# arielmission-space/PAOS

Measured on AMD Instinct MI355X. Metric: wavefronts/sec (4096^2 c128, 20-surface chain) + achieved HBM GB/s, higher is better.
Workload: dtype c128 (f64); 1 GPU; SYN20 20-surface chain (SURVEY 8d: 43 2-D FFTs per wavefront as the reference runs it), 4096x4096 fp64, walked 512-wavelength sweep, 32 wavefronts/GPU/step, PSFs stay in HBM; separable pass programs + ptp identities ([24] passes/wavefront, parity 1e-15..2e-14 vs oracle); grid=4096, batch_per_gpu=32, parallelism=wavefront-sharded x1, transport=none (single process), ranks_seen=1, launcher=none

## Files before the change

### include/paos_hip.h

```cpp
#ifndef PAOS_HIP_H
#define PAOS_HIP_H

#ifdef __cplusplus
extern "C" {
#endif

typedef struct paos_ctx paos_ctx;

enum { PAOS_OK = 0, PAOS_EINVAL = 1, PAOS_EHIP = 2, PAOS_EUNSUPPORTED = 3 };
enum { PAOS_F64 = 0, PAOS_F32 = 1 };
enum { PAOS_SHAPE_ELLIPSE = 0, PAOS_SHAPE_RECT = 1 };
enum { PAOS_KERNEL_PASS_ROWS = 0, PAOS_KERNEL_PASS_COLS = 1, PAOS_KERNEL_PASS_ANY = 2 };
enum { PAOS_PW_SIGN = 1, PAOS_PW_QPHASE_CENTRED = 2, PAOS_PW_QPHASE_NATURAL = 3, PAOS_PW_SCALE = 4,
       PAOS_PW_MASK = 5 };
enum { PAOS_PWF_MUL2PI = 1,
       PAOS_PWF_X_ONLY = 2, PAOS_PWF_Y_ONLY = 4 };
enum { PAOS_MAX_PW = 6 };
enum { PAOS_NORM_SLOTS = 64 };
enum { PAOS_WHAT_FIELD = 0, PAOS_WHAT_AMPLITUDE = 1, PAOS_WHAT_PHASE = 2, PAOS_WHAT_INTENSITY = 3 };

enum { PAOS_PHASE_STRIDE = 5 };
enum { PAOS_APERTURE_STRIDE = 8 };
enum { PAOS_ZERNIKE_HEAD = 8 };

// ... 75 lines not shown
int paos_focus_begin(paos_ctx* ctx);
int paos_focus_plane(paos_ctx* ctx, const double* params);
int paos_focus_end(paos_ctx* ctx);
enum { PAOS_OTF_MTF = 0, PAOS_OTF_COMPLEX = 1 };
int paos_otf_compute(paos_ctx* ctx);
int paos_otf_fetch(paos_ctx* ctx, int item, int what, void* host_out);
int paos_otf_cuts(paos_ctx* ctx, double* host_out);
int paos_zoom_weights(int n, int s, double frac, double* w, int* carry);
enum { PAOS_ZOOM_PSF = 0, PAOS_ZOOM_FIELD = 1 };
int paos_zoom_compute(paos_ctx* ctx, int m, int s, const double* centres, int want_field);
int paos_zoom_fetch(paos_ctx* ctx, int item, int what, void* host_out);
int paos_run_passes(paos_ctx* ctx, const paos_pass* passes, int n_passes, const double* blocks,
                    int n_blocks);
int paos_copy_yardstick(paos_ctx* ctx, int reps, double* ms_per_launch, double* bytes_per_launch);
int paos_record_set_stats(paos_ctx* ctx, unsigned long long* found, unsigned long long* rendered);
int paos_ctx_set_pruning(paos_ctx* ctx, int on);
int paos_run_passes_live(paos_ctx* ctx, const paos_pass* passes, int n_passes, const double* blocks,
                         int n_blocks, const double* live_rows);
int paos_run_program(paos_ctx* ctx, const paos_pass* passes, int n_passes, const double* blocks, int n_blocks,
                     const paos_program_opts* opts);
int paos_zernike(paos_ctx* ctx, int nmax, int kdim, const double* table, const double* params,
                 int param_stride, double* host_wfe);
int paos_zernike_like(paos_ctx* ctx, int nmax, int kdim, const double* table, const double* params,
                      int param_stride, const double* same_as, double* host_wfe);


int paos_pupil_aperture(paos_ctx* ctx, int shape, const double* params);
int paos_pupil_upload(paos_ctx* ctx, int item, const double* host_weights);
int paos_zernike_gram(paos_ctx* ctx, int nmax, int kdim, const double* table, const double* params,
                      int param_stride, int K, const double* poly, int use_pupil, double* host_out);
// ... 19 lines not shown
```

### paos_amd/_lib.py

```python
import ctypes
import os
import threading
import weakref

import numpy as np

_HERE = os.path.dirname(os.path.abspath(__file__))
LIB_PATH = os.environ.get("PAOS_LIB") or os.path.join(_HERE, "libpaoship.so")

PAOS_F64, PAOS_F32 = 0, 1
SHAPE_ELLIPSE, SHAPE_RECT = 0, 1
WHAT_FIELD, WHAT_AMPLITUDE, WHAT_PHASE, WHAT_INTENSITY = 0, 1, 2, 3
KERNEL_PASS_ROWS, KERNEL_PASS_COLS, KERNEL_PASS_ANY = 0, 1, 2
PW_SIGN, PW_QPHASE_CENTRED, PW_QPHASE_NATURAL, PW_SCALE, PW_MASK = 1, 2, 3, 4, 5
PWF_MUL2PI = 1
PWF_X_ONLY, PWF_Y_ONLY = 2, 4
MAX_PW = 6
OTF_MTF, OTF_COMPLEX = 0, 1
ZOOM_PSF, ZOOM_FIELD = 0, 1
ZOOM_MAX_TABLES = 256
NORM_SLOTS = 64


class PwOp(ctypes.Structure):
# ... 50 lines not shown
    "paos_ptp": (ctypes.c_int, [_c_ctx, _dbl_p]),
    "paos_stw": (ctypes.c_int, [_c_ctx, _dbl_p, ctypes.c_int]),
    "paos_wts": (ctypes.c_int, [_c_ctx, _dbl_p, ctypes.c_int]),
    "paos_focus_begin": (ctypes.c_int, [_c_ctx]),
    "paos_focus_plane": (ctypes.c_int, [_c_ctx, _dbl_p]),
    "paos_focus_end": (ctypes.c_int, [_c_ctx]),
    "paos_otf_compute": (ctypes.c_int, [_c_ctx]),
    "paos_otf_fetch": (ctypes.c_int, [_c_ctx, ctypes.c_int, ctypes.c_int, ctypes.c_void_p]),
    "paos_otf_cuts": (ctypes.c_int, [_c_ctx, _dbl_p]),
    "paos_zoom_weights": (ctypes.c_int, [ctypes.c_int, ctypes.c_int, ctypes.c_double, _dbl_p, ctypes.POINTER(ctypes.c_int)]),
    "paos_zoom_compute": (ctypes.c_int, [_c_ctx, ctypes.c_int, ctypes.c_int, _dbl_p, ctypes.c_int]),
    "paos_zoom_fetch": (ctypes.c_int, [_c_ctx, ctypes.c_int, ctypes.c_int, ctypes.c_void_p]),
    "paos_run_passes": (ctypes.c_int, [_c_ctx, ctypes.POINTER(Pass), ctypes.c_int, _dbl_p, ctypes.c_int]),
    "paos_copy_yardstick": (ctypes.c_int, [_c_ctx, ctypes.c_int, _dbl_p, _dbl_p]),
    "paos_record_set_stats": (ctypes.c_int, [_c_ctx, ctypes.POINTER(ctypes.c_ulonglong), ctypes.POINTER(ctypes.c_ulonglong)]),
    "paos_ctx_set_pruning": (ctypes.c_int, [_c_ctx, ctypes.c_int]),
    "paos_run_passes_live": (ctypes.c_int, [_c_ctx, ctypes.POINTER(Pass), ctypes.c_int, _dbl_p, ctypes.c_int, _dbl_p]),
    "paos_zernike": (ctypes.c_int, [_c_ctx, ctypes.c_int, ctypes.c_int, _dbl_p, _dbl_p, ctypes.c_int, _dbl_p]),
    "paos_psf_keep": (ctypes.c_int, [_c_ctx]),
    "paos_psf_keep_power": (ctypes.c_int, [_c_ctx, ctypes.POINTER(ctypes.c_int)]),
    "paos_psf_fetch": (ctypes.c_int, [_c_ctx, ctypes.c_int, _dbl_p]),
    "paos_host_alloc": (ctypes.c_int, [ctypes.c_ulonglong, ctypes.POINTER(ctypes.c_void_p)]),
    "paos_host_free": (ctypes.c_int, [ctypes.c_void_p]),
    "paos_export_pinned": (ctypes.c_int, [_c_ctx, ctypes.c_int, ctypes.c_int, ctypes.c_void_p]),
    "paos_start": (ctypes.c_int, [_c_ctx, ctypes.c_double, ctypes.c_double, ctypes.c_int, _dbl_p, _dbl_p]),
    "paos_pupil_aperture": (ctypes.c_int, [_c_ctx, ctypes.c_int, _dbl_p]),
    "paos_pupil_upload": (ctypes.c_int, [_c_ctx, ctypes.c_int, _dbl_p]),
    "paos_zernike_like": (ctypes.c_int, [_c_ctx, ctypes.c_int, ctypes.c_int, _dbl_p, _dbl_p, ctypes.c_int, _dbl_p, _dbl_p]),
    "paos_zernike_gram": (ctypes.c_int, [_c_ctx, ctypes.c_int, ctypes.c_int, _dbl_p, _dbl_p, ctypes.c_int,
                                         ctypes.c_int, _dbl_p, ctypes.c_int, _dbl_p]),
# ... 496 lines not shown
                                              out.ctypes.data_as(ctypes.c_void_p)), "paos_zoom_fetch")
        return out

    def copy_yardstick(self, reps=10):
        ms, nbytes = ctypes.c_double(0.0), ctypes.c_double(0.0)
        self._check(self._lib.paos_copy_yardstick(self._ctx, int(reps), ctypes.byref(ms), ctypes.byref(nbytes)),
                    "paos_copy_yardstick")
        return ms.value, nbytes.value

    def record_set_stats(self):
        found, rendered = ctypes.c_ulonglong(0), ctypes.c_ulonglong(0)
        self._check(self._lib.paos_record_set_stats(self._ctx, ctypes.byref(found), ctypes.byref(rendered)),
                    "paos_record_set_stats")
        return int(found.value), int(rendered.value)

    def set_pruning(self, on):
        self._check(self._lib.paos_ctx_set_pruning(self._ctx, 1 if on else 0), "paos_ctx_set_pruning")

    def run_passes(self, passes, blocks, live_rows=None, rows_stale=False, final_intensity=False, live_cols=None):
        b = np.ascontiguousarray(blocks, dtype=np.float64)
        if b.ndim != 3 or b.shape[1:] != (self.batch, PHASE_STRIDE):
            raise ValueError("blocks must be [n_blocks][batch][5]")
        arr = (Pass * len(passes))()
        for dst, src in zip(arr, passes):
            dst.axis, dst.fft1, dst.fft2 = src["axis"], src.get("fft1", -1), src.get("fft2", -1)
            for name in ("pre", "mid", "post"):
                ops = src.get(name, ())
                if len(ops) > MAX_PW:
                    raise ValueError("too many operators in one pass slot")
                setattr(dst, "n_" + name, len(ops))
# ... 108 lines not shown
```

### paos_amd/csrc/context.hip

```cpp
#include "host.h"

#include <cmath>
#include <complex>
#include <cstring>
#include <mutex>
#include <set>
#include <utility>

namespace {

thread_local std::string g_err;

}

int fail(paos_ctx* c, int code, const std::string& msg) {
  if (c) c->err = msg;
  g_err = msg;
  return code;
}

namespace {

int arena_switch(paos_ctx* c) {
  Arena& a = c->arena;
// ... 219 lines not shown
  c->device = device; c->n = n; c->batch = batch; c->precision = precision;
  const int bc = precision == PAOS_F64 ? Lay<double>::BC : Lay<float>::BC;
  c->br = (precision == PAOS_F32 && n >= 2048) ? PAOS_F32_BR : PAOS_BR;
  c->pitch = (unsigned)n * c->br + (unsigned)PAOS_PAD_BLOCKS * c->br * bc;
  c->item_stride = c->pitch * (unsigned)(n / c->br);
  const size_t eb = elem_bytes(c);
  auto bail = [&](hipError_t e, const char* what) {
    std::string msg = std::string(what) + ": " + hipGetErrorString(e);
    paos_ctx_destroy(c);
    return fail(nullptr, PAOS_EHIP, msg);
  };
  hipError_t e;
  if ((e = hipSetDevice(device)) != hipSuccess) return bail(e, "hipSetDevice");
  if ((e = hipStreamCreateWithFlags(&c->stream, hipStreamNonBlocking)) != hipSuccess) return bail(e, "hipStreamCreate");
  if (const char* pad = getenv("PAOS_LDS_PAD")) c->lds_pad = (size_t)std::max(0, std::atoi(pad));
  if ((e = hipMalloc(&c->dyn_scale, (size_t)batch * sizeof(double))) != hipSuccess) return bail(e, "hipMalloc(dyn_scale)");
  {
    std::vector<double> ones((size_t)batch, 1.0);
    if ((e = hipMemcpy(c->dyn_scale, ones.data(), ones.size() * sizeof(double), hipMemcpyHostToDevice)) != hipSuccess) return bail(e, "hipMemcpy(dyn_scale)");
  }
  if ((e = hipMalloc(&c->field, (size_t)c->item_stride * batch * eb)) != hipSuccess) return bail(e, "hipMalloc(field)");
  if ((e = hipMemsetAsync(c->field, 0, (size_t)c->item_stride * batch * eb, c->stream)) != hipSuccess) return bail(e, "hipMemset(field)");
  if ((e = hipMalloc(&c->tw, (size_t)n * eb)) != hipSuccess) return bail(e, "hipMalloc(tw)");
  if ((e = hipMalloc(&c->staging, (size_t)n * n * 16)) != hipSuccess) return bail(e, "hipMalloc(staging)");
  c->nparts = 1024;
  if ((e = hipMalloc(&c->partial, (size_t)batch * c->nparts * sizeof(double))) != hipSuccess) return bail(e, "hipMalloc(partial)");
  if ((e = hipMalloc(&c->norm2, (size_t)batch * sizeof(double))) != hipSuccess) return bail(e, "hipMalloc(norm2)");
  if ((e = hipHostMalloc(&c->norm2_host, (size_t)kNormSlots * batch * sizeof(double))) != hipSuccess) return bail(e, "hipHostMalloc(norm2)");
  c->arena.cap = (size_t)1 << 18;
  if (c->arena.cap < (size_t)batch * 2048) c->arena.cap = (size_t)batch * 2048;
// ... 165 lines not shown
}

int paos_norm2_release(paos_ctx* c, int ticket) {
  if (!c || ticket < 0 || ticket >= kNormSlots) return fail(c, PAOS_EINVAL, "bad ticket");
  c->norm_busy[ticket] = false;
  return PAOS_OK;
}

int paos_record_set_stats(paos_ctx* c, unsigned long long* found, unsigned long long* rendered) {
  if (!c || !found || !rendered) return fail(c, PAOS_EINVAL, "bad record-set request");
  *found = c->mask_hits;
  *rendered = c->mask_rendered;
  return PAOS_OK;
}

int paos_ctx_set_pruning(paos_ctx* c, int on) {
  if (!c) return fail(c, PAOS_EINVAL, "null context");
  c->prune = on != 0;
  return PAOS_OK;
}

}
```

### paos_amd/csrc/fft_core.h

```cpp
#pragma once
#include <hip/hip_runtime.h>

namespace paos {

template <typename T>
struct cx {
  T x, y;
};

template <typename T>
__device__ __forceinline__ cx<T> cadd(cx<T> a, cx<T> b) { return {a.x + b.x, a.y + b.y}; }
template <typename T>
__device__ __forceinline__ cx<T> csub(cx<T> a, cx<T> b) { return {a.x - b.x, a.y - b.y}; }
template <typename T>
__device__ __forceinline__ cx<T> cmul(cx<T> a, cx<T> b) {
  return {fma(a.x, b.x, -(a.y * b.y)), fma(a.x, b.y, a.y * b.x)};
}
template <typename T>
__device__ __forceinline__ cx<T> cconj(cx<T> a) { return {a.x, -a.y}; }
template <typename T>
__device__ __forceinline__ cx<T> sub_ib(cx<T> a, cx<T> b) { return {a.x + b.y, a.y - b.x}; }
template <typename T>
__device__ __forceinline__ cx<T> add_ib(cx<T> a, cx<T> b) { return {a.x - b.y, a.y + b.x}; }
template <typename T>
// ... 183 lines not shown
    dft<4, DIR>(b);
#pragma unroll
    for (int k2 = 0; k2 < 4; ++k2) v[4 * k2] = b[k2];
  }
  lf_twiddled_dft4<1, DIR>(y + 4, o);
#pragma unroll
  for (int k2 = 0; k2 < 4; ++k2) v[1 + 4 * k2] = o[k2];
  lf_twiddled_dft4<2, DIR>(y + 8, o);
#pragma unroll
  for (int k2 = 0; k2 < 4; ++k2) v[2 + 4 * k2] = o[k2];
  lf_twiddled_dft4<3, DIR>(y + 12, o);
#pragma unroll
  for (int k2 = 0; k2 < 4; ++k2) v[3 + 4 * k2] = o[k2];
}

template <int R, int DIR, typename T>
__device__ __forceinline__ void dft(cx<T>* v) {
  if constexpr (R == 16 && PAOS_LF16 != 0) {
    dft16_lf<DIR>(v);
  } else if constexpr (R == 2) {
    cx<T> a = v[0], b = v[1];
    v[0] = cadd(a, b);
    v[1] = csub(a, b);
  } else if constexpr (R == 4) {
    cx<T> t0 = cadd(v[0], v[2]), t1 = csub(v[0], v[2]);
    cx<T> t2 = cadd(v[1], v[3]), t3 = csub(v[1], v[3]);
    v[0] = cadd(t0, t2);
    v[2] = csub(t0, t2);
    if constexpr (DIR > 0) {
      v[1] = sub_ib(t1, t3);
// ... 89 lines not shown
#endif
#define PAOS_SYNC() do { if (!(PAOS_DIAG & 1)) __syncthreads(); } while (0)
#define PAOS_SYNC_X() do { if (!((PAOS_DIAG & 4) && NS > 1)) PAOS_SYNC(); } while (0)

#define PAOS_FENCE() do { if constexpr (FR != 0) __builtin_amdgcn_sched_barrier(0); } while (0)
#ifndef PAOS_NOFENCE
#define PAOS_NOFENCE 0
#endif
#define PAOS_FENCE_IF(bit) do { if constexpr (FR != 0 && !(PAOS_NOFENCE & (bit))) __builtin_amdgcn_sched_barrier(0); } while (0)
#ifndef PAOS_TAIL_FENCE
#define PAOS_TAIL_FENCE 1
#endif
#ifndef PAOS_TABLE_TWIDDLES
#define PAOS_TABLE_TWIDDLES 1
#endif
template <typename T, int N, int E, int DIR, bool SPLIT, int NS = 1, int FR = 0>
__device__ __forceinline__ void fft_stages(cx<T>* v, void* lds, int t,
                                           const cx<T>* __restrict__ tw, const cx<double>* circle = nullptr,
                                           const cx<T>* w1_last = nullptr) {
  using S = StageInfo<N, E, NS>;
  constexpr int TL = N / E;
  constexpr int R = S::R;
  constexpr int TPT = S::TPT;

#pragma unroll
  for (int s = 0; s < TPT; ++s) {
    if constexpr (NS > 1) {
      const int j = t + s * TL;
      const int k = j & (NS - 1);
      if constexpr (FR != 0 && PAOS_TABLE_TWIDDLES && sizeof(T) == 8 && NS * R == 256) {
        cx<double> wa = circle[k], wb = circle[2 * k];
// ... 1 lines not shown
        for (int r = 1; r < R; ++r) {
          const cx<double> w = wa;
          wa = wb;
          if (r + 2 < R) wb = circle[k * (r + 2)];
          v[s * R + r] = cmul(v[s * R + r], cx<T>{(T)w.x, (T)(DIR > 0 ? -w.y : w.y)});
          PAOS_FENCE_IF(4);
        }
      } else {
        cx<T> w1 = (w1_last != nullptr && NS * R == N) ? w1_last[s] : tw[k * (N / (NS * R))];
        if constexpr (DIR < 0) w1.y = -w1.y;
        if constexpr (FR != 0) apply_twiddle_chain<R>(v + s * R, w1);
        else apply_twiddle_powers<R>(v + s * R, w1);
      }
      PAOS_FENCE_IF(2);
    }
    if constexpr (!(((PAOS_DIAG & 8) && NS == 1) || ((PAOS_DIAG & 16) && S::LAST))) dft<R, DIR>(v + s * R);
    if constexpr (!(S::LAST && PAOS_TAIL_FENCE == 0)) PAOS_FENCE();
  }

  if constexpr (!S::LAST) {
    using SN = StageInfo<N, E, NS * R>;
    constexpr int R2 = SN::R;
    constexpr int TPT2 = SN::TPT;
    constexpr bool LIN_R = (TL % 16 == 0) && ((N / R2) % 16 == 0);
    int wb[TPT];
#pragma unroll
    for (int s = 0; s < TPT; ++s) {
      const int j = t + s * TL;
      wb[s] = lds_pad((j / NS) * (NS * R) + (j & (NS - 1)));
    }
    const int rb = lds_pad(t);
// ... 24 lines not shown
            if (!(PAOS_DIAG & 2)) l[wb[s] + lds_pad(r * NS)] = part ? v[s * R + r].y : v[s * R + r].x;
        PAOS_SYNC_X();
#pragma unroll
        for (int s = 0; s < TPT2; ++s)
#pragma unroll
          for (int r = 0; r < R2; ++r) {
            if (!(PAOS_DIAG & 2)) {
              const T val = l[ridx(s, r)];
              if (part) v[s * R2 + r].y = val; else v[s * R2 + r].x = val;
            }
          }
        if (part == 0 || !SN::LAST) PAOS_SYNC_X();
      }
    }
    PAOS_FENCE_IF(1);
    fft_stages<T, N, E, DIR, SPLIT, NS * R, FR>(v, lds, t, tw, circle, w1_last);
  }
}

constexpr int kSwapRow = 272;

__device__ __forceinline__ int swap_nibbles(int t) { return ((t & 15) << 4) | (t >> 4); }

template <typename T, bool BARRIER>
__device__ __forceinline__ void swap_exchange(cx<T>* v, T* lds, int wbase, int wstride, int rbase, int rstride, bool first) {
#pragma unroll
  for (int part = 0; part < 2; ++part) {
    if (BARRIER && (part == 1 || !first)) __syncthreads();
#pragma unroll
    for (int r = 0; r < 16; ++r) lds[wbase + r * wstride] = part ? v[r].y : v[r].x;
    if (BARRIER) __syncthreads();
// ... 75 lines not shown
```

### paos_amd/csrc/frugal_launch.h

```cpp
#pragma once
#include "host.h"

namespace {

#ifndef PAOS_LONG_ONE_LINE
#define PAOS_LONG_ONE_LINE 1
#endif
#ifndef PAOS_SINGLE_ONE_LINE
#define PAOS_SINGLE_ONE_LINE 1
#endif
template <typename T, int N, int AXIS, int KPRE, int KMID, int NFFT, int STORE = 0, int TAB = 0, int LONG = 0, int ONE = 0>
int frugal_launch(paos_ctx* c, const FrugalArgs& args) {
  using C = FftCfg<T, N>;
  constexpr bool kOneLine = PAOS_LONG_ONE_LINE != 0 && (LONG != 0 || ONE != 0) && STORE == 0 && sizeof(T) == 8 && N == 4096;
  constexpr int kOcc = (PAOS_LONG_ONE_LINE != 0 && (LONG != 0 || ONE != 0) && STORE == 0 && sizeof(T) == 8 && N == 2048) ? 1 : 0;
  constexpr int LINES = kOneLine ? 1 : (AXIS == 0 ? C::FR_ROW_LINES : C::COL_LINES);
  constexpr int TILES = AXIS == 0 ? C::ROW_TILES : C::COL_TILES;
  constexpr bool SPLIT = sizeof(T) == 8 || LINES > 2;
  FrugalArgs a = args;
  unsigned groups = N / LINES / TILES;
  a.wg0 = 0;
  constexpr unsigned kAlign = (kOneLine && AXIS == 0) ? 32 : 16;
  static_assert((N / LINES / TILES) % kAlign == 0, "TileMap renumbers tiles inside aligned groups of workgroups");
  if (a.live_hi > a.live_lo) {
    const unsigned per = LINES * TILES;
    a.wg0 = (a.live_lo / per) / kAlign * kAlign;
    unsigned end = ((a.live_hi + per - 1) / per + kAlign - 1) / kAlign * kAlign;
    if (end > groups) end = groups;
    groups = end - a.wg0;
  }
  const dim3 grid(groups, c->batch), block(TILES * LINES * N / C::E);
  constexpr size_t kMaxPad = 8192;
  const size_t lds = frugal_lds_bytes<T, N, LINES, TILES, SPLIT, KPRE, KMID, C::E, STORE, kOcc>() + (c->lds_pad < kMaxPad ? c->lds_pad : kMaxPad);
  auto kern = frugal_pass_kernel<T, N, C::E, LINES, TILES, AXIS, C::BR, C::BC, SPLIT, KPRE, KMID, NFFT, STORE, TAB, LONG, kOcc>;
  return TIMED_LAUNCH(c, kern, grid, block, lds, frugal_lds_bytes<T, N, LINES, TILES, SPLIT, KPRE, KMID, C::E, STORE, kOcc>() + kMaxPad,
                      AXIS == 0 ? PAOS_KERNEL_PASS_ROWS : PAOS_KERNEL_PASS_COLS, c->prof_next_tag, PAOS_FRUGAL_PASS(a));
}

template <typename T, int N, int AXIS, int KPRE, int KMID>
int frugal_nfft(paos_ctx* c, const FrugalArgs& a, int nfft) {
  if (a.tab && a.fuse) {
    if constexpr (KPRE == 1 && KMID == 1) {
      if (nfft < 2) return fail(c, PAOS_EINVAL, "a fused chain starts with a two-transform pass");
#define PAOS_LONG_CASE(L)                                                           \
  case L:                                                                           \
    if (a.psf) return frugal_launch<T, N, AXIS, 1, 1, 2, 1, 1, L>(c, a);            \
    if (a.pow_partial) return frugal_launch<T, N, AXIS, 1, 1, 2, 2, 1, L>(c, a);    \
    return frugal_launch<T, N, AXIS, 1, 1, 2, 0, 1, L>(c, a);
      switch (a.fuse) {
        PAOS_LONG_CASE(1)
        PAOS_LONG_CASE(2)
        PAOS_LONG_CASE(3)
        PAOS_LONG_CASE(4)
      }
#undef PAOS_LONG_CASE
      return fail(c, PAOS_EINVAL, "a launch runs at most three passes");
    } else {
      return fail(c, PAOS_EINVAL, "no fused build of this pass shape");
    }
  }
  if (a.tab) {
    if constexpr (KPRE <= 1 && KMID <= 1 && KPRE + KMID > 0) {
      if (a.psf) return nfft >= 2 ? frugal_launch<T, N, AXIS, KPRE, KMID, 2, 1, 1>(c, a) : frugal_launch<T, N, AXIS, KPRE, KMID, 1, 1, 1>(c, a);
      if (a.pow_partial) return nfft >= 2 ? frugal_launch<T, N, AXIS, KPRE, KMID, 2, 2, 1>(c, a) : frugal_launch<T, N, AXIS, KPRE, KMID, 1, 2, 1>(c, a);
      if constexpr (sizeof(T) == 8 && (N == 4096 || N == 2048) && PAOS_LONG_ONE_LINE != 0) {
        if (a.one_line && PAOS_SINGLE_ONE_LINE != 0) return nfft >= 2 ? frugal_launch<T, N, AXIS, KPRE, KMID, 2, 0, 1, 0, 1>(c, a) : frugal_launch<T, N, AXIS, KPRE, KMID, 1, 0, 1, 0, 1>(c, a);
      }
      return nfft >= 2 ? frugal_launch<T, N, AXIS, KPRE, KMID, 2, 0, 1>(c, a) : frugal_launch<T, N, AXIS, KPRE, KMID, 1, 0, 1>(c, a);
    } else {
      return fail(c, PAOS_EINVAL, "no table build of this pass shape");
    }
  }
  if constexpr (KPRE <= 1 && KMID <= 1) {
    if (a.psf) return nfft >= 2 ? frugal_launch<T, N, AXIS, KPRE, KMID, 2, 1>(c, a) : frugal_launch<T, N, AXIS, KPRE, KMID, 1, 1>(c, a);
  } else {
    if (a.psf) return fail(c, PAOS_EUNSUPPORTED, "no PSF-storing build of this pass shape");
  }
  if constexpr (KPRE <= 1) {
    if (a.pow_partial) return nfft >= 2 ? frugal_launch<T, N, AXIS, KPRE, KMID, 2, 2>(c, a) : frugal_launch<T, N, AXIS, KPRE, KMID, 1, 2>(c, a);
  } else {
// ... 28 lines not shown
```

### paos_amd/csrc/frugal_pass.h

```cpp
#pragma once
#include "fft_kernels.h"

#ifndef PAOS_FENCE_EVERY
#define PAOS_FENCE_EVERY 2
#endif
#ifndef PAOS_PRIO_LOAD
#define PAOS_PRIO_LOAD 0
#endif
#ifndef PAOS_PRIO_STORE
#define PAOS_PRIO_STORE 0
#endif
#ifndef PAOS_PREFETCH
#define PAOS_PREFETCH 0
#endif

namespace paos {

constexpr int kFrugalMaxPre = 2, kFrugalMaxMid = 3;

struct FrugalPhase {
  double sx, sy, coef, sgn, m2, natural;
};
constexpr int kMaskW = 192;
struct MaskLine {
// ... 32 lines not shown
  void* field;
  const void* tw;
  const FrugalItem* items;
  unsigned pitch, item_stride;
  double* psf;
  double* psf_partial;
  double* pow_partial;
  const double* dyn_scale;
#if PAOS_STAMPS
  unsigned long long* stamps;
#endif
  unsigned live_lo, live_hi, wg0;
  int tab = 0;
  int fuse = 0;
  int one_line = 0;
};
#if PAOS_STAMPS
#define PAOS_STAMP(i)                                                                              \
  do {                                                                                             \
    if (threadIdx.x == 0)                                                                          \
      a.stamps[((size_t)blockIdx.y * gridDim.x + blockIdx.x) * kStampSlots + (i)] = __builtin_amdgcn_s_memtime(); \
  } while (0)
#define PAOS_STAMP_WAIT_VM() asm volatile("s_waitcnt vmcnt(0)" ::: "memory")
#else
#define PAOS_STAMP(i) do { } while (0)
#define PAOS_STAMP_WAIT_VM() do { } while (0)
#endif

constexpr int kCircleLds = 256;
template <bool TAIL = false>
// ... 93 lines not shown
    const double e = __dadd_rn(__dsub_rn(q0, __dsub_rn(a, bb)), __dsub_rn(q1, bb));
    const float frac = turn_fraction(a) + (float)(e * 0.15915494309189535);
    return cx<float>{__builtin_amdgcn_cosf(frac), __builtin_amdgcn_sinf(frac)};
  }
#pragma unroll
  for (int j = 0; j < K; ++j) {
    const double x = __dmul_rn(g[j], step[j]);
    const double q = __dmul_rn(m2[j], __dmul_rn(coefq[j], __dadd_rn(__dmul_rn(x, x), across2[j])));
    const float frac = turn_fraction(q);
    const float snf = __builtin_amdgcn_sinf(frac), csf = __builtin_amdgcn_cosf(frac);
    p = j == 0 ? cx<float>{csf, snf} : cmul_after_trans(p, cx<float>{csf, snf});
  }
  return p;
}

template <typename T, int N, int E, int K, typename Map, int PLAIN = 0, bool SHARE = false, int RECS = 0, int TAB = 0>
__device__ __forceinline__ void frugal_slot(cx<T>* v, const FrugalSlot& sl, const FrugalPhase* ph,
                                            const Map& m, const cx<double>* circle, bool conj_in, bool conj_out, int tpos,
                                            void* area = nullptr, bool area_busy = false, const MaskLine* recs = nullptr,
                                            int lbase = 0, double extra_scale = 1.0) {
  if constexpr (PLAIN == 1) {
    static_assert(K == 0, "a plain slot has no phases");
    const unsigned mask = (conj_out != conj_in) ? 0x80000000u : 0u;
#pragma unroll
    for (int k = 0; k < E; ++k) v[k].y = flip_sign(v[k].y, mask);
    return;
  }
  if constexpr (PLAIN == 2) {
    static_assert(K == 0, "a plain slot has no phases");
    const unsigned mask = (conj_out != conj_in) ? 0x80000000u : 0u;
    const unsigned none = (sl.sign_on != 0.0) ? 0x80000000u : 0u;
#pragma unroll
    for (int k = 0; k < E; ++k) {
      v[k].x = flip_sign(v[k].x, none);
      v[k].y = flip_sign(v[k].y, mask);
      if ((k + 1) % PAOS_FENCE_EVERY == 0) __builtin_amdgcn_sched_barrier(0);
    }
    return;
  }
  constexpr int TL = N / E;
  static_assert(TL % 2 == 0, "the checkerboard sign is constant along a thread's elements");
  const double sc = __dmul_rn(sl.scale, extra_scale);
  const int line = Map::kAxis == 0 ? m.row(0) : m.col(0);
  if (sl.mask_on != 0.0) {
    MaskLine ml;
    if constexpr (RECS > 0) {
      ml = recs[0];
#pragma unroll
      for (int j = 1; j < RECS; ++j)
        if (line - lbase == j) ml = recs[j];
    } else if constexpr (RECS < 0) {
      ml = recs[line - lbase];
    } else {
      ml = sl.lines[line];
    }
    constexpr int R = (kMaskW + TL - 1) / TL;
// ... 5 lines not shown
    double wa[R], wb[R];
    int sel_a[R], sel_b[R];
#pragma unroll
    for (int j = 0; j < R; ++j) {
      const int pa = tpos + (ka + j) * TL, pb = tpos + (kb + j) * TL;
      const bool hit_a = ka + j < E && pa < ml.p1, hit_b = kb + j < E && pb < ml.p3;
      wa[j] = val(hit_a ? pa - ml.p0 : 0);
      wb[j] = val(hit_b ? kMaskW + pb - ml.p2 : kMaskW);
      sel_a[j] = hit_a ? ka + j : -1;
      sel_b[j] = hit_b ? kb + j : -1;
    }
    const double w_in = __dmul_rn(sl.w_in, ml.lm), w_out = __dmul_rn(sl.w_out, ml.lm);
#pragma unroll
    for (int j = 0; j < R; ++j) { wa[j] = __dmul_rn(wa[j], ml.lm); wb[j] = __dmul_rn(wb[j], ml.lm); }
#pragma unroll
    for (int k = 0; k < E; ++k) {
      const int pos = tpos + k * TL;
      double w = (pos >= ml.p1 && pos < ml.p2) ? w_in : w_out;
#pragma unroll
      for (int j = 0; j < R; ++j) {
        w = (k == sel_a[j]) ? wa[j] : w;
        w = (k == sel_b[j]) ? wb[j] : w;
      }
      if constexpr (sizeof(T) == 4) {
        const float wf = (float)w;
        v[k] = {(T)(v[k].x * wf), (T)(v[k].y * wf)};
      } else {
        v[k] = {(T)__dmul_rn((double)v[k].x, w), (T)__dmul_rn((double)v[k].y, w)};
      }
      if ((k + 1) % PAOS_FENCE_EVERY == 0) __builtin_amdgcn_sched_barrier(0);
    }
// ... 84 lines not shown
    return slot_factor<K>(gk, step, across2, coefq, m2s, circle);
  };
  auto apply = [&](int k, cx<double> p) __attribute__((always_inline)) {
    const cx<double> vd = {(double)v[k].x, (double)v[k].y};
#if defined(PAOS_DIAG_NOSCALE)
    v[k] = {(T)(fma(vd.x, p.x, -(vd.y * p.y))), (T)(fma(vd.x, p.y, vd.y * p.x))};
#else
    v[k] = {(T)(fma(vd.x, p.x, -(vd.y * p.y)) * f), (T)(fma(vd.x, p.y, vd.y * p.x) * fy)};
#endif
  };
  if constexpr (K > 0 && TAB != 0) {
    static_assert(!SHARE, "a table slot does not stand for a barrier");
    const cx<double>* tb = sl.table + tpos;
    constexpr int kFence = Map::kLinesPerWorkgroup == 1 ? 4 : PAOS_TABLE_FENCE;
#pragma unroll
    for (int k = 0; k < E; ++k) {
#if defined(PAOS_DIAG_NOTABLE)
      apply(k, cx<double>{0.6, 0.8});
#else
      apply(k, tb[k * TL]);
#endif
      if ((k + 1) % kFence == 0) __builtin_amdgcn_sched_barrier(0);
    }
    return;
  }
  if constexpr (SHARE && K > 0) {
    cx<double>* fac = reinterpret_cast<cx<double>*>(area);
    if (area_busy) lds_barrier();
#pragma unroll
    for (int k = 0; k < E / 2; ++k) {
      const cx<double> p = factor(k);
      fac[k * TL + tpos] = p;
      apply(k, p);
      if ((k + 1) % PAOS_FENCE_EVERY == 0) __builtin_amdgcn_sched_barrier(0);
    }
    if (tpos == 0) fac[(E / 2) * TL] = factor(E / 2);
    lds_barrier();
// ... 70 lines not shown
  typedef T vec2 __attribute__((ext_vector_type(2)));
  if constexpr (NT) {
    const vec2 t = __builtin_nontemporal_load(reinterpret_cast<const vec2*>(p));
    return {t.x, t.y};
  } else {
    return *p;
  }
}
template <bool NT, typename T>
__device__ __forceinline__ void stream_store(cx<T>* p, cx<T> v) {
  typedef T vec2 __attribute__((ext_vector_type(2)));
  if constexpr (NT) __builtin_nontemporal_store(vec2{v.x, v.y}, reinterpret_cast<vec2*>(p));
  else *p = v;
}

template <typename T, int N, int E, bool SPLIT, bool FLIP = true>
__device__ __forceinline__ void frugal_fft(cx<T>* v, void* lds, int t, const cx<T>* tw, const cx<double>* circle,
                                           double inv, const cx<T>* w1_last = nullptr) {
  fft_stages<T, N, E, +1, SPLIT, 1, 1>(v, lds, t, tw, circle, w1_last);
  unpermute_slots<N, E>(v);
  if constexpr (FLIP) {
    const unsigned mask = inv != 0.0 ? 0x80000000u : 0u;
#pragma unroll
    for (int k = 0; k < E; ++k) v[k].y = flip_sign(v[k].y, mask);
  }
  if constexpr (!(FLIP && PAOS_TAIL_FENCE == 0)) __builtin_amdgcn_sched_barrier(0);
}

constexpr size_t kStoreScratch = 16 * sizeof(double);
#ifndef PAOS_HOIST_RECORDS
#define PAOS_HOIST_RECORDS 1
#endif
template <int LINES, int TILES, int KPRE>
constexpr int frugal_record_mode() {
// ... 49 lines not shown
    *out = s;
  }
}

#if PAOS_STAMPS
#define PAOS_FRUGAL_PARAMS const FrugalItem *k_items, void *k_field, unsigned k_pitch, unsigned k_item_stride, unsigned k_wg0, \
                           const void *k_tw, double *k_psf, double *k_psf_partial, double *k_pow_partial, const double *k_dyn_scale, \
                           unsigned long long *k_stamps
#define PAOS_FRUGAL_PASS(a) (a).items, (a).field, (a).pitch, (a).item_stride, (a).wg0, (a).tw, (a).psf, (a).psf_partial, (a).pow_partial, (a).dyn_scale, (a).stamps
#else
#define PAOS_FRUGAL_PARAMS const FrugalItem *k_items, void *k_field, unsigned k_pitch, unsigned k_item_stride, unsigned k_wg0, \
                           const void *k_tw, double *k_psf, double *k_psf_partial, double *k_pow_partial, const double *k_dyn_scale
#define PAOS_FRUGAL_PASS(a) (a).items, (a).field, (a).pitch, (a).item_stride, (a).wg0, (a).tw, (a).psf, (a).psf_partial, (a).pow_partial, (a).dyn_scale
#endif
template <typename T, int N, int E, int LINES, int TILES, int AXIS, int BR, int BC, bool SPLIT,
          int KPRE, int KMID, int NFFT, int STORE = 0, int TAB = 0, int LONG = 0, int OCC = 0>
__global__ void __launch_bounds__(TILES* LINES* N / E, (frugal_min_waves<T, N, TILES * LINES * N / E, OCC>()))
    frugal_pass_kernel(PAOS_FRUGAL_PARAMS) {
  static_assert(LONG == 0 || (TAB != 0 && (NFFT == 2 || NFFT == 3) && KPRE == 1 && KMID == 1), "LONG builds: see above");
  FrugalArgs a;
  a.items = k_items; a.field = k_field; a.pitch = k_pitch; a.item_stride = k_item_stride; a.wg0 = k_wg0;
  a.tw = k_tw; a.psf = k_psf; a.psf_partial = k_psf_partial; a.pow_partial = k_pow_partial; a.dyn_scale = k_dyn_scale; a.live_lo = a.live_hi = 0;
#if PAOS_STAMPS
  a.stamps = k_stamps;
#endif
  const int item = blockIdx.y;
  typedef const __attribute__((address_space(4))) FrugalItem* ConstItemPtr;
  const FrugalItem& it = *(const FrugalItem*)((ConstItemPtr)a.items + item);
  constexpr int kThreads = TILES * LINES * N / E;
  constexpr int kTwiddleLds = twiddle_lds_entries<N, E>();
  constexpr int kTwIt = (kTwiddleLds + kThreads - 1) / kThreads;
  constexpr int kClIt = sizeof(T) == 8 ? (kCircleLds + kThreads - 1) / kThreads : 1;
  constexpr int kExtra = (LONG + 1) / 2;
  const FrugalItem& it_last = LONG == 0 ? it : *(const FrugalItem*)((ConstItemPtr)a.items + item + kExtra * gridDim.y);
// ... 87 lines not shown
  unsigned pf_sink = 0;
  if constexpr (PAOS_PREFETCH > 0) {
    const unsigned wgp = wg + (unsigned)PAOS_PREFETCH;
    if (wgp < a.wg0 + gridDim.x) {
      const TileMap<N, E, LINES, TILES, AXIS, BR, BC, 1, COLSIB, kSwz> mp(wgp, threadIdx.x & ~3u, a.pitch);
      typedef const __attribute__((address_space(1))) char* GlobalBytes;
      const GlobalBytes pbase = (GlobalBytes)fb;
#pragma unroll
      for (int j = 0; j < E / 4; ++j) {
        const unsigned off = (mp.base + (unsigned)(4 * j + (threadIdx.x & 3)) * mp.stride) * (unsigned)sizeof(cx<T>);
        asm volatile("global_load_dword %0, %1, %2" : "+v"(pf_sink) : "v"(off), "s"(pbase) : "memory");
      }
      __builtin_amdgcn_sched_barrier(0);
    }
  }
  if (plo <= 0 && phi >= N) {
#pragma unroll
    for (int k = 0; k < E; ++k) v[k] = stream_load<NTL>(at(k));
  } else {
#pragma unroll
    for (int k = 0; k < E; ++k) {
      const int pos = m.t + k * (N / E);
      v[k] = cx<T>{(T)0, (T)0};
      if (pos >= plo && pos < phi) v[k] = stream_load<NTL>(at(k));
    }
  }
  __builtin_amdgcn_sched_barrier(0);
  cx<T> tw_fetch[kTwIt], cl_fetch[kClIt];
  constexpr int kRecDwords = kRecMode == 1 ? TILES * LINES * (int)(sizeof(MaskLine) / 4) : 0;
  static_assert(kRecDwords <= 128, "the record area is filled by the first 128 threads");
  const bool stage_recs = kRecMode == 1 && h_mask_on != 0.0;
// ... 83 lines not shown
        for (int k = 0; k < E; ++k) stream_store<NT>(at(k), v[k]);
      } else {
#pragma unroll
        for (int k = 0; k < E; ++k) {
          const int pos = m.t + k * (N / E);
          if (pos >= slo3 && pos < shi3) stream_store<NT>(at(k), v[k]);
        }
      }
    }
    return;
  }
  const bool ran1 = it.fft1_on != 0.0;
  const bool ran2 = NFFT == 2 && it.fft2_on != 0.0;
  const bool inv1 = ran1 && it.fft1_inv != 0.0;
  constexpr bool kShare = PAOS_SHARE_PHASES != 0 && TAB == 0;
  frugal_slot<T, N, E, KPRE, decltype(m), kPlainPre, kShare && KMID == 0, 0, TAB>(v, it.pre, it.pre_ph, m, circle, false, inv1, m.t, lds, false);
  PAOS_STAMP(2);
  if (ran1) frugal_fft<T, N, E, SPLIT, false>(v, lds, m.t, tw, circle, it.fft1_inv, w1_last);
  PAOS_STAMP(3);
  constexpr bool kShareMid = kShare && KPRE == 0 && KMID < 3;
  frugal_slot<T, N, E, KMID, decltype(m), 0, kShareMid, (kRecMode == 1 ? -1 : kRecs), TAB>(
      v, it.mid, it.mid_ph, m, circle, inv1, ran2 && it.fft2_inv != 0.0, m.t, lds, ran1, kRecMode == 1 ? rec_lds : mrec, lbase, h_dyn);
  PAOS_STAMP(4);
  if constexpr (NFFT == 2) {
    if (ran2) {
      if (ran1 && !(kShareMid && KMID > 0)) __syncthreads();
      frugal_fft<T, N, E, SPLIT>(v, lds, m.t, tw, circle, it.fft2_inv, w1_last);
    }
  }
  if constexpr (LONG != 0) {
    bool busy = ran1 || ran2;
#define PAOS_EXTRA_PASS(ix, kTwo)                                                                                                    \
  {                                                                                                                                  \
// ... 77 lines not shown
```

### paos_amd/csrc/host.h

```cpp
#pragma once
#include "../../include/paos_hip.h"

#include <hip/hip_runtime.h>

#include <cstdlib>
#include <string>
#include <type_traits>
#include <vector>

#include "frugal_pass.h"

using namespace paos;

#ifndef PAOS_BR
#define PAOS_BR 4
#endif
#ifndef PAOS_PAD_BLOCKS
#define PAOS_PAD_BLOCKS 3
#endif
inline constexpr int BR = PAOS_BR;
#ifndef PAOS_F32_BR
#define PAOS_F32_BR 8
#endif
template <typename T, int N>
// ... 76 lines not shown
  double* metric_partial = nullptr;
  double* metric_out = nullptr;
  double* metric_host = nullptr;
  struct MaskSet {
    MaskLine* lines = nullptr;
    double* vals = nullptr;
    std::vector<double> key;
    unsigned long long used = 0;
    int line_lo = 0, line_hi = 0;
  };
  static constexpr int kMaskSets = 8;
  MaskSet mask_sets[kMaskSets];
  unsigned long long mask_clock = 0;
  unsigned long long mask_hits = 0, mask_rendered = 0;
  size_t lds_pad = 0;
  int* mask_overflow = nullptr;
  double* partial = nullptr;
  double* norm2 = nullptr;
  double* norm2_host = nullptr;
  bool prune = true;
  int norm_slot = 0;
  bool norm_busy[64] = {};
  int nparts = 0;
  Arena arena;
  std::string err;
  int prof_kind = -1;
  std::vector<hipEvent_t> prof_events;
  std::vector<int> prof_tags;
  int prof_next_tag = 0;
  double prof_next_bytes = 0.0;
// ... 137 lines not shown
```

### paos_amd/csrc/passes.hip

```cpp
#include "host.h"

#include <algorithm>
#include <cmath>
#include <cstdio>
#include <cstring>

#include "phase_tables.h"

namespace {

int check_ops(paos_ctx* c, const paos_pw_op* ops, int count, int n_blocks) {
  if (count < 0 || count > PAOS_MAX_PW) return fail(c, PAOS_EINVAL, "too many pointwise operators in a pass");
  for (int o = 0; o < count; ++o) {
    if (ops[o].kind < PAOS_PW_SIGN || ops[o].kind > PAOS_PW_MASK) return fail(c, PAOS_EINVAL, "unknown pointwise operator");
    if (ops[o].block < 0 || ops[o].block >= n_blocks) return fail(c, PAOS_EINVAL, "operator block index out of range");
    if (ops[o].kind == PAOS_PW_MASK && ops[o].block + 1 >= n_blocks) return fail(c, PAOS_EINVAL, "an aperture operator needs two parameter blocks");
  }
  return PAOS_OK;
}

bool use_tables() {
  static const bool on = env_is("PAOS_PHASE_TABLES", '1');
  return on;
}
// ... 235 lines not shown
    for (const LoweredPass* l : {(const LoweredPass*)&lp, (const LoweredPass*)next, (const LoweredPass*)next2}) {
      if (!l) continue;
      const FrugalItem& fk = l->items[it];
      c->prof_next_lines += (fi.line_hi - fi.line_lo) * ((fk.fft1_on != 0.0 ? 1.0 : 0.0) + (l->nfft >= 2 && fk.fft2_on != 0.0 ? 1.0 : 0.0));
    }
  }
  a.tab = tables ? 1 : 0;
  {
    bool light = tables && !next && !store_psf && !sum_power;
    for (int it = 0; it < c->batch && light; ++it) {
      const FrugalItem& fi = lp.items[it];
      if (fi.active == 0.0) continue;
      light = 2.0 * (fi.pos_hi - fi.pos_lo) <= (double)c->n && 2.0 * (fi.spos_hi - fi.spos_lo) <= (double)c->n;
    }
    a.one_line = light ? 1 : 0;
  }
  a.fuse = next2 ? 2 + next2->nfft : (next ? next->nfft : 0);
  const int kpre = next ? 1 : (tables && lp.kpre > 1 ? 1 : lp.kpre), kmid = next ? 1 : (tables && lp.kmid > 1 ? 1 : lp.kmid);
  if (c->precision == PAOS_F64) {
    switch (c->n) {
      case 1024: return paos_frugal_d1024(c, a, p.axis, kpre, kmid, nfft);
      case 2048: return paos_frugal_d2048(c, a, p.axis, kpre, kmid, nfft);
      default: return paos_frugal_d4096(c, a, p.axis, kpre, kmid, nfft);
    }
  }
  switch (c->n) {
    case 2048: return paos_frugal_f2048(c, a, p.axis, kpre, kmid, nfft);
    default: return paos_frugal_f4096(c, a, p.axis, kpre, kmid, nfft);
  }
}
// ... 445 lines not shown
```

Before: 2182 wavefronts/s.

## Add central-half specialised pass kernels that skip zero outer quarters of input lines

When every active item's live input span lies within the central half of the line, a new kernel variant loads only the middle half of each thread's elements, applies pre-slot table operators only to those, and uses a pruned first radix-16 butterfly that assumes the outer inputs are zero. It is meant to cut input reads, pointwise work and first-stage FFT arithmetic for padded pupils. It is enabled by default (PAOS_CENTRAL_HALF env can disable it) and adds more template instantiations, plus launch counters for statistics.

```diff
diff --git a/include/paos_hip.h b/include/paos_hip.h
--- a/include/paos_hip.h
+++ b/include/paos_hip.h
@@ -113,6 +113,7 @@
                     int n_blocks);
 int paos_copy_yardstick(paos_ctx* ctx, int reps, double* ms_per_launch, double* bytes_per_launch);
 int paos_record_set_stats(paos_ctx* ctx, unsigned long long* found, unsigned long long* rendered);
+int paos_central_half_stats(paos_ctx* ctx, unsigned long long* central, unsigned long long* plain);
 int paos_ctx_set_pruning(paos_ctx* ctx, int on);
 int paos_run_passes_live(paos_ctx* ctx, const paos_pass* passes, int n_passes, const double* blocks,
                          int n_blocks, const double* live_rows);
diff --git a/paos_amd/_lib.py b/paos_amd/_lib.py
--- a/paos_amd/_lib.py
+++ b/paos_amd/_lib.py
@@ -88,6 +88,7 @@
     "paos_run_passes": (ctypes.c_int, [_c_ctx, ctypes.POINTER(Pass), ctypes.c_int, _dbl_p, ctypes.c_int]),
     "paos_copy_yardstick": (ctypes.c_int, [_c_ctx, ctypes.c_int, _dbl_p, _dbl_p]),
     "paos_record_set_stats": (ctypes.c_int, [_c_ctx, ctypes.POINTER(ctypes.c_ulonglong), ctypes.POINTER(ctypes.c_ulonglong)]),
+    "paos_central_half_stats": (ctypes.c_int, [_c_ctx, ctypes.POINTER(ctypes.c_ulonglong), ctypes.POINTER(ctypes.c_ulonglong)]),
     "paos_ctx_set_pruning": (ctypes.c_int, [_c_ctx, ctypes.c_int]),
     "paos_run_passes_live": (ctypes.c_int, [_c_ctx, ctypes.POINTER(Pass), ctypes.c_int, _dbl_p, ctypes.c_int, _dbl_p]),
     "paos_zernike": (ctypes.c_int, [_c_ctx, ctypes.c_int, ctypes.c_int, _dbl_p, _dbl_p, ctypes.c_int, _dbl_p]),
@@ -614,6 +615,12 @@
                     "paos_record_set_stats")
         return int(found.value), int(rendered.value)
 
+    def central_half_stats(self):
+        central, plain = ctypes.c_ulonglong(0), ctypes.c_ulonglong(0)
+        self._check(self._lib.paos_central_half_stats(self._ctx, ctypes.byref(central), ctypes.byref(plain)),
+                    "paos_central_half_stats")
+        return int(central.value), int(plain.value)
+
     def set_pruning(self, on):
         self._check(self._lib.paos_ctx_set_pruning(self._ctx, 1 if on else 0), "paos_ctx_set_pruning")
 
diff --git a/paos_amd/csrc/context.hip b/paos_amd/csrc/context.hip
--- a/paos_amd/csrc/context.hip
+++ b/paos_amd/csrc/context.hip
@@ -257,6 +257,8 @@
   if ((e = hipSetDevice(device)) != hipSuccess) return bail(e, "hipSetDevice");
   if ((e = hipStreamCreateWithFlags(&c->stream, hipStreamNonBlocking)) != hipSuccess) return bail(e, "hipStreamCreate");
   if (const char* pad = getenv("PAOS_LDS_PAD")) c->lds_pad = (size_t)std::max(0, std::atoi(pad));
+  if (env_is("PAOS_CENTRAL_HALF", '0')) c->central_half = false;
+  if (env_is("PAOS_CENTRAL_HALF", '1')) c->central_half = true;
   if ((e = hipMalloc(&c->dyn_scale, (size_t)batch * sizeof(double))) != hipSuccess) return bail(e, "hipMalloc(dyn_scale)");
   {
     std::vector<double> ones((size_t)batch, 1.0);
@@ -452,6 +454,13 @@
   return PAOS_OK;
 }
 
+int paos_central_half_stats(paos_ctx* c, unsigned long long* central, unsigned long long* plain) {
+  if (!c || !central || !plain) return fail(c, PAOS_EINVAL, "bad central-half request");
+  *central = c->central_launches;
+  *plain = c->plain_launches;
+  return PAOS_OK;
+}
+
 int paos_ctx_set_pruning(paos_ctx* c, int on) {
   if (!c) return fail(c, PAOS_EINVAL, "null context");
   c->prune = on != 0;
diff --git a/paos_amd/csrc/fft_core.h b/paos_amd/csrc/fft_core.h
--- a/paos_amd/csrc/fft_core.h
+++ b/paos_amd/csrc/fft_core.h
@@ -221,6 +221,37 @@
   for (int k2 = 0; k2 < 4; ++k2) v[3 + 4 * k2] = o[k2];
 }
 
+template <int DIR, typename T>
+__device__ __forceinline__ void dft16_lf_central(cx<T>* v) {
+  static_assert(DIR > 0, "the pass kernel runs forward transforms only");
+  cx<T> y[16];
+#pragma unroll
+  for (int n2 = 0; n2 < 4; ++n2) {
+    const cx<T> a = v[4 + n2], b = v[8 + n2];
+    const cx<T> nb = {-b.x, -b.y};
+    y[0 * 4 + n2] = cadd(b, a);
+    y[1 * 4 + n2] = sub_ib(nb, a);
+    y[2 * 4 + n2] = csub(b, a);
+    y[3 * 4 + n2] = add_ib(nb, a);
+  }
+  cx<T> o[4];
+  {
+    cx<T> b[4] = {y[0], y[1], y[2], y[3]};
+    dft<4, DIR>(b);
+#pragma unroll
+    for (int k2 = 0; k2 < 4; ++k2) v[4 * k2] = b[k2];
+  }
+  lf_twiddled_dft4<1, DIR>(y + 4, o);
+#pragma unroll
+  for (int k2 = 0; k2 < 4; ++k2) v[1 + 4 * k2] = o[k2];
+  lf_twiddled_dft4<2, DIR>(y + 8, o);
+#pragma unroll
+  for (int k2 = 0; k2 < 4; ++k2) v[2 + 4 * k2] = o[k2];
+  lf_twiddled_dft4<3, DIR>(y + 12, o);
+#pragma unroll
+  for (int k2 = 0; k2 < 4; ++k2) v[3 + 4 * k2] = o[k2];
+}
+
 template <int R, int DIR, typename T>
 __device__ __forceinline__ void dft(cx<T>* v) {
   if constexpr (R == 16 && PAOS_LF16 != 0) {
@@ -340,7 +371,7 @@
 #ifndef PAOS_TABLE_TWIDDLES
 #define PAOS_TABLE_TWIDDLES 1
 #endif
-template <typename T, int N, int E, int DIR, bool SPLIT, int NS = 1, int FR = 0>
+template <typename T, int N, int E, int DIR, bool SPLIT, int NS = 1, int FR = 0, int CH = 0>
 __device__ __forceinline__ void fft_stages(cx<T>* v, void* lds, int t,
                                            const cx<T>* __restrict__ tw, const cx<double>* circle = nullptr,
                                            const cx<T>* w1_last = nullptr) {
@@ -372,7 +403,10 @@
       }
       PAOS_FENCE_IF(2);
     }
-    if constexpr (!(((PAOS_DIAG & 8) && NS == 1) || ((PAOS_DIAG & 16) && S::LAST))) dft<R, DIR>(v + s * R);
+    if constexpr (CH != 0 && NS == 1 && PAOS_LF16 != 0) {
+      static_assert(R == 16 && TPT == 1, "central-half first stage: one 16-point butterfly per thread");
+      dft16_lf_central<DIR>(v);
+    } else if constexpr (!(((PAOS_DIAG & 8) && NS == 1) || ((PAOS_DIAG & 16) && S::LAST))) dft<R, DIR>(v + s * R);
     if constexpr (!(S::LAST && PAOS_TAIL_FENCE == 0)) PAOS_FENCE();
   }
 
@@ -427,7 +461,7 @@
       }
     }
     PAOS_FENCE_IF(1);
-    fft_stages<T, N, E, DIR, SPLIT, NS * R, FR>(v, lds, t, tw, circle, w1_last);
+    fft_stages<T, N, E, DIR, SPLIT, NS * R, FR, 0>(v, lds, t, tw, circle, w1_last);
   }
 }
 
diff --git a/paos_amd/csrc/frugal_launch.h b/paos_amd/csrc/frugal_launch.h
--- a/paos_amd/csrc/frugal_launch.h
+++ b/paos_amd/csrc/frugal_launch.h
@@ -9,9 +9,12 @@
 #ifndef PAOS_SINGLE_ONE_LINE
 #define PAOS_SINGLE_ONE_LINE 1
 #endif
-template <typename T, int N, int AXIS, int KPRE, int KMID, int NFFT, int STORE = 0, int TAB = 0, int LONG = 0, int ONE = 0>
+template <typename T, int N, int KPRE, int TAB>
+constexpr bool frugal_central() { return sizeof(T) == 8 && N == 4096 && KPRE == 1 && TAB != 0; }
+template <typename T, int N, int AXIS, int KPRE, int KMID, int NFFT, int STORE = 0, int TAB = 0, int LONG = 0, int ONE = 0, int CH = 0>
 int frugal_launch(paos_ctx* c, const FrugalArgs& args) {
   using C = FftCfg<T, N>;
+  static_assert(CH == 0 || frugal_central<T, N, KPRE, TAB>(), "no central-half build of this shape");
   constexpr bool kOneLine = PAOS_LONG_ONE_LINE != 0 && (LONG != 0 || ONE != 0) && STORE == 0 && sizeof(T) == 8 && N == 4096;
   constexpr int kOcc = (PAOS_LONG_ONE_LINE != 0 && (LONG != 0 || ONE != 0) && STORE == 0 && sizeof(T) == 8 && N == 2048) ? 1 : 0;
   constexpr int LINES = kOneLine ? 1 : (AXIS == 0 ? C::FR_ROW_LINES : C::COL_LINES);
@@ -32,7 +35,8 @@
   const dim3 grid(groups, c->batch), block(TILES * LINES * N / C::E);
   constexpr size_t kMaxPad = 8192;
   const size_t lds = frugal_lds_bytes<T, N, LINES, TILES, SPLIT, KPRE, KMID, C::E, STORE, kOcc>() + (c->lds_pad < kMaxPad ? c->lds_pad : kMaxPad);
-  auto kern = frugal_pass_kernel<T, N, C::E, LINES, TILES, AXIS, C::BR, C::BC, SPLIT, KPRE, KMID, NFFT, STORE, TAB, LONG, kOcc>;
+  auto kern = frugal_pass_kernel<T, N, C::E, LINES, TILES, AXIS, C::BR, C::BC, SPLIT, KPRE, KMID, NFFT, STORE, TAB, LONG, kOcc, CH>;
+  ++(CH != 0 ? c->central_launches : c->plain_launches);
   return TIMED_LAUNCH(c, kern, grid, block, lds, frugal_lds_bytes<T, N, LINES, TILES, SPLIT, KPRE, KMID, C::E, STORE, kOcc>() + kMaxPad,
                       AXIS == 0 ? PAOS_KERNEL_PASS_ROWS : PAOS_KERNEL_PASS_COLS, c->prof_next_tag, PAOS_FRUGAL_PASS(a));
 }
@@ -44,6 +48,9 @@
       if (nfft < 2) return fail(c, PAOS_EINVAL, "a fused chain starts with a two-transform pass");
 #define PAOS_LONG_CASE(L)                                                           \
   case L:                                                                           \
+    if constexpr (frugal_central<T, N, 1, 1>() && PAOS_LONG_ONE_LINE != 0) {   \
+      if (a.central && !a.psf && !a.pow_partial) return frugal_launch<T, N, AXIS, 1, 1, 2, 0, 1, L, 0, 1>(c, a);  \
+    }                                                                               \
     if (a.psf) return frugal_launch<T, N, AXIS, 1, 1, 2, 1, 1, L>(c, a);            \
     if (a.pow_partial) return frugal_launch<T, N, AXIS, 1, 1, 2, 2, 1, L>(c, a);    \
     return frugal_launch<T, N, AXIS, 1, 1, 2, 0, 1, L>(c, a);
@@ -64,6 +71,10 @@
       if (a.psf) return nfft >= 2 ? frugal_launch<T, N, AXIS, KPRE, KMID, 2, 1, 1>(c, a) : frugal_launch<T, N, AXIS, KPRE, KMID, 1, 1, 1>(c, a);
       if (a.pow_partial) return nfft >= 2 ? frugal_launch<T, N, AXIS, KPRE, KMID, 2, 2, 1>(c, a) : frugal_launch<T, N, AXIS, KPRE, KMID, 1, 2, 1>(c, a);
       if constexpr (sizeof(T) == 8 && (N == 4096 || N == 2048) && PAOS_LONG_ONE_LINE != 0) {
+        if constexpr (frugal_central<T, N, KPRE, 1>()) {
+          if (a.one_line && a.central && PAOS_SINGLE_ONE_LINE != 0)
+            return nfft >= 2 ? frugal_launch<T, N, AXIS, KPRE, KMID, 2, 0, 1, 0, 1, 1>(c, a) : frugal_launch<T, N, AXIS, KPRE, KMID, 1, 0, 1, 0, 1, 1>(c, a);
+        }
         if (a.one_line && PAOS_SINGLE_ONE_LINE != 0) return nfft >= 2 ? frugal_launch<T, N, AXIS, KPRE, KMID, 2, 0, 1, 0, 1>(c, a) : frugal_launch<T, N, AXIS, KPRE, KMID, 1, 0, 1, 0, 1>(c, a);
       }
       return nfft >= 2 ? frugal_launch<T, N, AXIS, KPRE, KMID, 2, 0, 1>(c, a) : frugal_launch<T, N, AXIS, KPRE, KMID, 1, 0, 1>(c, a);
diff --git a/paos_amd/csrc/frugal_pass.h b/paos_amd/csrc/frugal_pass.h
--- a/paos_amd/csrc/frugal_pass.h
+++ b/paos_amd/csrc/frugal_pass.h
@@ -70,6 +70,7 @@
   int tab = 0;
   int fuse = 0;
   int one_line = 0;
+  int central = 0;
 };
 #if PAOS_STAMPS
 #define PAOS_STAMP(i)                                                                              \
@@ -193,7 +194,7 @@
   return p;
 }
 
-template <typename T, int N, int E, int K, typename Map, int PLAIN = 0, bool SHARE = false, int RECS = 0, int TAB = 0>
+template <typename T, int N, int E, int K, typename Map, int PLAIN = 0, bool SHARE = false, int RECS = 0, int TAB = 0, int CH = 0>
 __device__ __forceinline__ void frugal_slot(cx<T>* v, const FrugalSlot& sl, const FrugalPhase* ph,
                                             const Map& m, const cx<double>* circle, bool conj_in, bool conj_out, int tpos,
                                             void* area = nullptr, bool area_busy = false, const MaskLine* recs = nullptr,
@@ -219,6 +220,8 @@
   }
   constexpr int TL = N / E;
   static_assert(TL % 2 == 0, "the checkerboard sign is constant along a thread's elements");
+  static_assert(CH == 0 || (K > 0 && TAB != 0 && sizeof(T) == 8 && E % 4 == 0), "central-half slots: complex128 table slots");
+  constexpr int kFirst = CH != 0 ? E / 4 : 0, kEnd = CH != 0 ? 3 * E / 4 : E;
   const double sc = __dmul_rn(sl.scale, extra_scale);
   const int line = Map::kAxis == 0 ? m.row(0) : m.col(0);
   if (sl.mask_on != 0.0) {
@@ -254,7 +257,7 @@
 #pragma unroll
     for (int j = 0; j < R; ++j) { wa[j] = __dmul_rn(wa[j], ml.lm); wb[j] = __dmul_rn(wb[j], ml.lm); }
 #pragma unroll
-    for (int k = 0; k < E; ++k) {
+    for (int k = kFirst; k < kEnd; ++k) {
       const int pos = tpos + k * TL;
       double w = (pos >= ml.p1 && pos < ml.p2) ? w_in : w_out;
 #pragma unroll
@@ -369,13 +372,13 @@
     const cx<double>* tb = sl.table + tpos;
     constexpr int kFence = Map::kLinesPerWorkgroup == 1 ? 4 : PAOS_TABLE_FENCE;
 #pragma unroll
-    for (int k = 0; k < E; ++k) {
+    for (int k = kFirst; k < kEnd; ++k) {
 #if defined(PAOS_DIAG_NOTABLE)
       apply(k, cx<double>{0.6, 0.8});
 #else
       apply(k, tb[k * TL]);
 #endif
-      if ((k + 1) % kFence == 0) __builtin_amdgcn_sched_barrier(0);
+      if ((k - kFirst + 1) % kFence == 0) __builtin_amdgcn_sched_barrier(0);
     }
     return;
   }
@@ -476,10 +479,10 @@
   else *p = v;
 }
 
-template <typename T, int N, int E, bool SPLIT, bool FLIP = true>
+template <typename T, int N, int E, bool SPLIT, bool FLIP = true, int CH = 0>
 __device__ __forceinline__ void frugal_fft(cx<T>* v, void* lds, int t, const cx<T>* tw, const cx<double>* circle,
                                            double inv, const cx<T>* w1_last = nullptr) {
-  fft_stages<T, N, E, +1, SPLIT, 1, 1>(v, lds, t, tw, circle, w1_last);
+  fft_stages<T, N, E, +1, SPLIT, 1, 1, CH>(v, lds, t, tw, circle, w1_last);
   unpermute_slots<N, E>(v);
   if constexpr (FLIP) {
     const unsigned mask = inv != 0.0 ? 0x80000000u : 0u;
@@ -559,10 +562,11 @@
 #define PAOS_FRUGAL_PASS(a) (a).items, (a).field, (a).pitch, (a).item_stride, (a).wg0, (a).tw, (a).psf, (a).psf_partial, (a).pow_partial, (a).dyn_scale
 #endif
 template <typename T, int N, int E, int LINES, int TILES, int AXIS, int BR, int BC, bool SPLIT,
-          int KPRE, int KMID, int NFFT, int STORE = 0, int TAB = 0, int LONG = 0, int OCC = 0>
+          int KPRE, int KMID, int NFFT, int STORE = 0, int TAB = 0, int LONG = 0, int OCC = 0, int CH = 0>
 __global__ void __launch_bounds__(TILES* LINES* N / E, (frugal_min_waves<T, N, TILES * LINES * N / E, OCC>()))
     frugal_pass_kernel(PAOS_FRUGAL_PARAMS) {
   static_assert(LONG == 0 || (TAB != 0 && (NFFT == 2 || NFFT == 3) && KPRE == 1 && KMID == 1), "LONG builds: see above");
+  static_assert(CH == 0 || (sizeof(T) == 8 && N == 4096 && E == 16 && TAB != 0 && KPRE == 1 && NFFT <= 2), "CH builds: see above");
   FrugalArgs a;
   a.items = k_items; a.field = k_field; a.pitch = k_pitch; a.item_stride = k_item_stride; a.wg0 = k_wg0;
   a.tw = k_tw; a.psf = k_psf; a.psf_partial = k_psf_partial; a.pow_partial = k_pow_partial; a.dyn_scale = k_dyn_scale; a.live_lo = a.live_hi = 0;
@@ -680,7 +684,15 @@
       __builtin_amdgcn_sched_barrier(0);
     }
   }
-  if (plo <= 0 && phi >= N) {
+  if constexpr (CH != 0) {
+#pragma unroll
+    for (int k = 0; k < E; ++k) v[k] = cx<T>{(T)0, (T)0};
+#pragma unroll
+    for (int k = E / 4; k < 3 * E / 4; ++k) {
+      const int pos = m.t + k * (N / E);
+      if (pos >= plo && pos < phi) v[k] = stream_load<NTL>(at(k));
+    }
+  } else if (plo <= 0 && phi >= N) {
 #pragma unroll
     for (int k = 0; k < E; ++k) v[k] = stream_load<NTL>(at(k));
   } else {
@@ -794,9 +806,9 @@
   const bool ran2 = NFFT == 2 && it.fft2_on != 0.0;
   const bool inv1 = ran1 && it.fft1_inv != 0.0;
   constexpr bool kShare = PAOS_SHARE_PHASES != 0 && TAB == 0;
-  frugal_slot<T, N, E, KPRE, decltype(m), kPlainPre, kShare && KMID == 0, 0, TAB>(v, it.pre, it.pre_ph, m, circle, false, inv1, m.t, lds, false);
+  frugal_slot<T, N, E, KPRE, decltype(m), kPlainPre, kShare && KMID == 0, 0, TAB, CH>(v, it.pre, it.pre_ph, m, circle, false, inv1, m.t, lds, false);
   PAOS_STAMP(2);
-  if (ran1) frugal_fft<T, N, E, SPLIT, false>(v, lds, m.t, tw, circle, it.fft1_inv, w1_last);
+  if (ran1) frugal_fft<T, N, E, SPLIT, false, CH>(v, lds, m.t, tw, circle, it.fft1_inv, w1_last);
   PAOS_STAMP(3);
   constexpr bool kShareMid = kShare && KPRE == 0 && KMID < 3;
   frugal_slot<T, N, E, KMID, decltype(m), 0, kShareMid, (kRecMode == 1 ? -1 : kRecs), TAB>(
diff --git a/paos_amd/csrc/host.h b/paos_amd/csrc/host.h
--- a/paos_amd/csrc/host.h
+++ b/paos_amd/csrc/host.h
@@ -114,6 +114,8 @@
   unsigned long long mask_clock = 0;
   unsigned long long mask_hits = 0, mask_rendered = 0;
   size_t lds_pad = 0;
+  bool central_half = true;
+  unsigned long long central_launches = 0, plain_launches = 0;
   int* mask_overflow = nullptr;
   double* partial = nullptr;
   double* norm2 = nullptr;
diff --git a/paos_amd/csrc/passes.hip b/paos_amd/csrc/passes.hip
--- a/paos_amd/csrc/passes.hip
+++ b/paos_amd/csrc/passes.hip
@@ -273,6 +273,16 @@
       light = 2.0 * (fi.pos_hi - fi.pos_lo) <= (double)c->n && 2.0 * (fi.spos_hi - fi.spos_lo) <= (double)c->n;
     }
     a.one_line = light ? 1 : 0;
+  }
+  {
+    bool central = c->central_half && tables, any = false;
+    for (int it = 0; it < c->batch && central; ++it) {
+      const FrugalItem& fi = lp.items[it];
+      if (fi.active == 0.0) continue;
+      any = true;
+      central = 4.0 * fi.pos_lo >= (double)c->n && 4.0 * fi.pos_hi <= 3.0 * (double)c->n;
+    }
+    a.central = central && any ? 1 : 0;
   }
   a.fuse = next2 ? 2 + next2->nfft : (next ? next->nfft : 0);
   const int kpre = next ? 1 : (tables && lp.kpre > 1 ? 1 : lp.kpre), kmid = next ? 1 : (tables && lp.kmid > 1 ? 1 : lp.kmid);
```

Result: faster. 2254 wavefronts/s (median of 6 runs) (+3.3%).
